# theblackcat102/edgedict

Hardware: NVIDIA H100
Metric: audio-sec/sec E6D2 B=32 T=1000 U=128 V=1024 training step (higher is better)
Workload: dtype bf16

## Files before the change

edgedict_b200/_lib.py:

```python
import ctypes as C
import os

_HERE = os.path.dirname(os.path.abspath(__file__))
LIB_PATH = os.path.join(_HERE, "libedgedict_b200.so")

_lib = None

P, I, L, F, D, Z = C.c_void_p, C.c_int, C.c_long, C.c_float, C.c_double, C.c_size_t

OPT_MAX_GROUPS = 16


class OptHyper(C.Structure):
    _fields_ = [(k, D * OPT_MAX_GROUPS) for k in ("lr", "wd", "b1", "b2", "eps")]


SIGNATURES = {
    "eb_rnnt_workspace_bytes": (Z, [I, I, I, I]),
    "eb_rnnt_loss_fwd": (I, [P, P, P, P, I, I, I, I, I, I, P, P, I, P]),
    "eb_rnnt_loss_bwd": (I, [P, P, I, P, P, P, I, I, I, I, I, I, P, P, I, D, P]),
    "eb_rnnt_loss_lattice": (I, [P, P, I, I, I, P, P, I, P]),
    "eb_rnnt_loss_bwd_bf16": (I, [P, P, P, P, P, I, I, I, I, I, P, P, I, D, P]),
    "eb_joint_logits_lse": (I, [P, P, P, P, P, P, P, P, P, P, I, I, I, I, I, I, P]),
    "eb_lm_logits_ce": (I, [P, P, P, P, P, I, P, P, L, I, I, P]),
    "eb_lm_ce_rows": (I, [P, P, I, P, P, L, I, P]),
    "eb_lm_ce_loss": (I, [P, P, P, I, L, L, I, I, P, P, P, P]),
    "eb_lm_ce_bwd": (I, [P, P, I, P, P, I, L, L, I, P, I, P, P]),
    "eb_rnnt_workspace_views": (I, [P, I, I, I, I, P, P, P, P, P]),
    "eb_rnnt_align_bytes": (Z, [I, I, I]),
    "eb_rnnt_viterbi": (I, [P, P, I, I, I, I, P, P, P, P, P, P]),
    "eb_log_softmax_fwd": (I, [P, P, L, I, P]),
    "eb_log_softmax_bwd": (I, [P, P, P, L, I, P]),
    "eb_ctc_workspace_size": (Z, [I, I, I]),
    "eb_ctc_loss_fwd": (I, [P, L, L, I, I, I, P, L, P, P, P, I, I, I, P, P, P]),
    "eb_ctc_loss_bwd": (I, [P, L, L, P, L, L, I, I, I, P, P, I, I, I, P, P, P]),
    "eb_ctc_greedy": (I, [P, L, L, I, I, I, P, I, P, P, P, P]),
    "eb_ctc_align_workspace_size": (Z, [I, I, I]),
    "eb_ctc_align": (I, [P, L, L, I, I, I, P, L, P, P, P, I, I, P, P, P, P]),
    "eb_gemm_f32": (I, [P, L, L, P, L, L, P, L, P, I, I, I, F, F, P]),
    "eb_gemm_bf16": (I, [P, I, P, I, P, I, P, I, L, I, L, P]),
    "eb_gemm_bf16_ex": (I, [P, I, P, I, P, I, P, I, L, I, L, I, P, L, P]),
    "eb_gemm_bf16_partials": (L, [I, I, I, L, I, L, I]),
    "eb_gemm_bf16_dtanh": (I, [P, I, P, I, P, P, L, I, L, P]),
    "eb_gemm_tc_set_trace": (I, [P, I]),
    "eb_joint_dpre_reduce": (I, [P, P, P, I, I, I, I, P]),
    "eb_lstm_scratch_bytes": (Z, [I, I]),
    "eb_lstm_seq_fwd": (I, [P, P, P, P, P, P, P, P, P, P, I, I, I, P]),
    "eb_lstm_seq_bwd": (I, [P, P, P, P, P, P, P, P, P, P, P, I, I, I, P]),
    "eb_gru_scratch_bytes": (Z, [I, I]),
    "eb_gru_seq_fwd": (I, [P, P, P, P, P, P, P, P, I, I, I, P]),
    "eb_gru_seq_bwd": (I, [P, P, P, P, P, P, P, P, P, P, I, I, I, P]),
    "eb_gru_tc_supported": (I, [I, I]),
    "eb_gru_tc_scratch_bytes": (Z, [I, I]),
    "eb_gru_tc_fwd": (I, [P, P, P, P, P, P, P, P, I, I, I, P]),
    "eb_gru_tc_bwd": (I, [P, P, P, P, P, P, P, P, P, P, I, I, I, P]),
# ... 103 lines not shown
```

edgedict_b200/csrc/common.cuh:

```cuda
#pragma once
#include <cuda_runtime.h>
#include <cuda_bf16.h>
#include <stdint.h>
#include <stdio.h>
#include <math.h>

#define EB_OK 0
#define EB_ERR_INVALID 2
#define EB_ERR_CUDA 3

#define EB_API extern "C" __attribute__((visibility("default")))

#define EB_CHECK_LAUNCH()                                                             \
    do {                                                                              \
        cudaError_t e__ = cudaGetLastError();                                         \
        if (e__ != cudaSuccess) {                                                     \
            fprintf(stderr, "[edgedict_b200] %s:%d CUDA error: %s\n", __FILE__,       \
                    __LINE__, cudaGetErrorString(e__));                               \
            return EB_ERR_CUDA;                                                       \
        }                                                                             \
    } while (0)

#define EB_CUDA(call)                                                                 \
    do {                                                                              \
// ... 50 lines not shown
    const int lane = threadIdx.x & 31, w = threadIdx.x >> 5;
    v = warp_sum(v);
    __syncthreads();
    if (lane == 0) sh[w] = v;
    __syncthreads();
    const int nw = (blockDim.x + 31) >> 5;
    T r = (threadIdx.x < nw) ? sh[threadIdx.x] : T(0);
    if (w == 0) {
        r = warp_sum(r);
        if (lane == 0) sh[32] = r;
    }
    __syncthreads();
    return sh[32];
}

__device__ __forceinline__ void spin_wait_ge(const unsigned* ctr, unsigned target) {
    unsigned v;
    long long t0 = 0;
    unsigned spins = 0;
    while (true) {
        asm volatile("ld.acquire.gpu.global.u32 %0, [%1];" : "=r"(v) : "l"(ctr) : "memory");
        if (v >= target) break;
        if ((++spins & 0xFFFF) == 0) {
            const long long now = clock64();
            if (t0 == 0) t0 = now;
            else if (now - t0 > 8000000000LL) {
                printf("[edgedict_b200] grid barrier timeout: block %d saw %u, wants %u\n", blockIdx.x, v, target);
                __trap();
            }
        }
    }
}

__device__ __forceinline__ float fast_ex2(float x) {
    float y;
    asm("ex2.approx.ftz.f32 %0, %1;" : "=f"(y) : "f"(x));
    return y;
}
__device__ __forceinline__ float fast_exp(float x) { return fast_ex2(x * 1.4426950408889634f); }
__device__ __forceinline__ float sigmoidf_(float x) { return 1.0f / (1.0f + expf(-x)); }

__device__ __forceinline__ float4 ld_stream_f4(const float* p) {
    float4 r;
    asm volatile("ld.global.nc.L1::no_allocate.v4.f32 {%0,%1,%2,%3}, [%4];"
                 : "=f"(r.x), "=f"(r.y), "=f"(r.z), "=f"(r.w) : "l"(p));
    return r;
}
__device__ __forceinline__ void st_stream_f4(float* p, float4 v) {
    asm volatile("st.global.L1::no_allocate.v4.f32 [%0], {%1,%2,%3,%4};"
                 :: "l"(p), "f"(v.x), "f"(v.y), "f"(v.z), "f"(v.w) : "memory");
}
```

edgedict_b200/csrc/elementwise.cu:

```cuda
#include <cooperative_groups.h>
#include "common.cuh"
#include "../../include/edgedict_b200.h"

namespace cg = cooperative_groups;

namespace {

constexpr int LN_WARPS = 8;

template <int PL>
__global__ void __launch_bounds__(LN_WARPS * 32)
layernorm_fwd_kernel(const float* __restrict__ x, const float* __restrict__ res,
                     const float* __restrict__ gamma, const float* __restrict__ beta,
                     float* __restrict__ y, __nv_bfloat16* __restrict__ y16,
                     float* __restrict__ mean, float* __restrict__ rstd, long rows, int H, float eps) {
    const int lane = threadIdx.x & 31;
    const long wstride = (long)gridDim.x * LN_WARPS;
    for (long r = (long)blockIdx.x * LN_WARPS + (threadIdx.x >> 5); r < rows; r += wstride) {
        const float* xr = x + r * H;
        const float* rr = res ? res + r * H : nullptr;
        float v[PL];
        float s = 0.f;
#pragma unroll
        for (int i = 0; i < PL; ++i) {
// ... 382 lines not shown
                acc[2 * i] += gf.x;
                acc[2 * i + 1] += gf.y;
            }
        }
        float* o = ddp + ((long)b * U + u) * J + q * 8;
        *reinterpret_cast<float4*>(o) = make_float4(acc[0], acc[1], acc[2], acc[3]);
        *reinterpret_cast<float4*>(o + 4) = make_float4(acc[4], acc[5], acc[6], acc[7]);
    }
}

template <int RL, int CW>
__device__ __forceinline__ float colsum_tree(float (*sh)[CW + 1], float v, int k, int cx) {
    sh[k][cx] = v;
    __syncthreads();
#pragma unroll 1
    for (int st = RL / 2; st > 0; st >>= 1) {
        if (k < st) sh[k][cx] += sh[k + st][cx];
        __syncthreads();
    }
    return sh[0][cx];
}
template <typename TI>
__global__ void __launch_bounds__(1024) colsum_kernel(const TI* __restrict__ x, float* __restrict__ out, long rows, int N) {
    __shared__ float sh[32][33];
    const int cx = threadIdx.x & 31, k = threadIdx.x >> 5;
    const int c = blockIdx.x * 32 + cx;
    float acc = 0.f;
    if (c < N)
        for (long r = k; r < rows; r += 32) acc += (float)x[r * N + c];
    const float t = colsum_tree<32, 32>(sh, acc, k, cx);
    if (k == 0 && c < N) out[c] += t;
}

constexpr int COLSUM_LANES = 512, COLSUM_CL = 4, COLSUM_CTA_LANES = COLSUM_LANES / COLSUM_CL;
__global__ void __cluster_dims__(1, COLSUM_CL, 1) __launch_bounds__(2 * COLSUM_CTA_LANES)
colsum_bf16_vec_kernel(const __nv_bfloat16* __restrict__ x, float* __restrict__ out, long rows, int N) {
    __shared__ float sh[COLSUM_CTA_LANES][17];
    cg::cluster_group cluster = cg::this_cluster();
    const unsigned rank = cluster.block_rank();
    const int half = threadIdx.x & 1, kl = threadIdx.x >> 1, k = (int)rank * COLSUM_CTA_LANES + kl;
    const int c0 = blockIdx.x * 16 + half * 8;
    float acc[8] = {0.f, 0.f, 0.f, 0.f, 0.f, 0.f, 0.f, 0.f};
    if (c0 < N) {
        const __nv_bfloat16* p = x + (long)k * N + c0;
        const long step = (long)COLSUM_LANES * N;
        long r = k;
        for (; r + 7 * COLSUM_LANES < rows; r += 8 * COLSUM_LANES) {
            uint4 v[8];
#pragma unroll
            for (int q = 0; q < 8; ++q) v[q] = *reinterpret_cast<const uint4*>(p + q * step);
#pragma unroll
            for (int q = 0; q < 8; ++q) {
                const uint32_t w[4] = {v[q].x, v[q].y, v[q].z, v[q].w};
#pragma unroll
                for (int i = 0; i < 4; ++i) {
                    const float2 f = __bfloat1622float2(*reinterpret_cast<const __nv_bfloat162*>(&w[i]));
                    acc[2 * i] += f.x;
                    acc[2 * i + 1] += f.y;
                }
            }
            p += 8 * step;
        }
        for (; r < rows; r += COLSUM_LANES, p += step) {
            const uint4 v = *reinterpret_cast<const uint4*>(p);
            const uint32_t w[4] = {v.x, v.y, v.z, v.w};
#pragma unroll
            for (int i = 0; i < 4; ++i) {
                const float2 f = __bfloat1622float2(*reinterpret_cast<const __nv_bfloat162*>(&w[i]));
                acc[2 * i] += f.x;
                acc[2 * i + 1] += f.y;
            }
        }
    }
#pragma unroll
    for (int i = 0; i < 8; ++i) sh[kl][half * 8 + i] = acc[i];
    cluster.sync();
    if (rank < 2) {
        const float* peer = cluster.map_shared_rank(&sh[0][0], rank + 2);
        for (int e = threadIdx.x; e < COLSUM_CTA_LANES * 16; e += blockDim.x) sh[e >> 4][e & 15] += peer[(e >> 4) * 17 + (e & 15)];
    }
    cluster.sync();
    if (rank == 0) {
        const float* peer = cluster.map_shared_rank(&sh[0][0], 1);
        for (int e = threadIdx.x; e < COLSUM_CTA_LANES * 16; e += blockDim.x) sh[e >> 4][e & 15] += peer[(e >> 4) * 17 + (e & 15)];
    }
    cluster.sync();
    if (rank != 0) return;
#pragma unroll 1
    for (int st = COLSUM_CTA_LANES / 2; st > 0; st >>= 1) {
        for (int e = threadIdx.x; e < st * 16; e += blockDim.x) sh[e >> 4][e & 15] += sh[(e >> 4) + st][e & 15];
        __syncthreads();
    }
    if (threadIdx.x < 16 && blockIdx.x * 16 + (int)threadIdx.x < N) out[blockIdx.x * 16 + threadIdx.x] += sh[0][threadIdx.x];
}

__global__ void cast_bf16_kernel(const float* __restrict__ x, __nv_bfloat16* __restrict__ y, long n) {
    long i = ((long)blockIdx.x * blockDim.x + threadIdx.x) * 4;
    const long stride = (long)gridDim.x * blockDim.x * 4;
    for (; i + 3 < n; i += stride) {
        float4 v = *reinterpret_cast<const float4*>(x + i);
        __nv_bfloat162 a = __floats2bfloat162_rn(v.x, v.y), b = __floats2bfloat162_rn(v.z, v.w);
        uint2 q;
        q.x = *reinterpret_cast<uint32_t*>(&a);
        q.y = *reinterpret_cast<uint32_t*>(&b);
        *reinterpret_cast<uint2*>(y + i) = q;
    }
    if (i < n) for (long k = i; k < n && k < i + 4; ++k) y[k] = __float2bfloat16(x[k]);
}

template <typename TI>
__global__ void transpose_to_bf16_kernel(const TI* __restrict__ x, __nv_bfloat16* __restrict__ y,
                                         long rows, long cols) {
    __shared__ float tile[32][33];
    const long c0 = (long)blockIdx.x * 32;
    for (long r0 = (long)blockIdx.y * 32; r0 < rows; r0 += (long)gridDim.y * 32) {
        for (int i = threadIdx.y; i < 32; i += blockDim.y) {
            long r = r0 + i, c = c0 + threadIdx.x;
            tile[i][threadIdx.x] = (r < rows && c < cols) ? (float)x[r * cols + c] : 0.f;
        }
        __syncthreads();
        for (int i = threadIdx.y; i < 32; i += blockDim.y) {
            long c = c0 + i, r = r0 + threadIdx.x;
            if (r < rows && c < cols) y[c * rows + r] = __float2bfloat16(tile[threadIdx.x][i]);
        }
        __syncthreads();
    }
// ... 199 lines not shown
    } else {
        joint_hidden_bwd_t_f32_kernel<<<B * T, 256, 0, ST(stream)>>>(
            (float*)dhidden_inout, (const float*)hidden, dep, T, U, J);
        EB_CHECK_LAUNCH();
        joint_hidden_bwd_u_f32_kernel<<<B * U, 256, 0, ST(stream)>>>((const float*)dhidden_inout, ddp, T, U, J);
    }
    EB_CHECK_LAUNCH();
    return EB_OK;
}

EB_API int eb_joint_dpre_reduce(const void* dpre16, float* dep, float* ddp, int B, int T, int U, int J, void* stream) {
    if (!dpre16 || !dep || !ddp || B <= 0 || T <= 0 || U <= 0 || J <= 0 || J % 8 ||
        ((reinterpret_cast<uintptr_t>(dpre16) | reinterpret_cast<uintptr_t>(dep) | reinterpret_cast<uintptr_t>(ddp)) & 15))
        return EB_ERR_INVALID;
    joint_dep_reduce_bf16_kernel<<<B * T, 96, 0, ST(stream)>>>((const __nv_bfloat16*)dpre16, dep, U, J);
    EB_CHECK_LAUNCH();
    joint_hidden_bwd_u_bf16_kernel<<<B * U, 96, 0, ST(stream)>>>((const __nv_bfloat16*)dpre16, ddp, T, U, J);
    EB_CHECK_LAUNCH();
    return EB_OK;
}

EB_API int eb_colsum(const void* x, int x_bf16, float* out, long rows, int N, void* stream) {
    if (!x || !out || rows <= 0 || N <= 0) return EB_ERR_INVALID;
    if (x_bf16 && N % 8 == 0 && (reinterpret_cast<uintptr_t>(x) & 15) == 0)
        colsum_bf16_vec_kernel<<<dim3((N + 15) / 16, COLSUM_CL), 2 * COLSUM_CTA_LANES, 0, ST(stream)>>>((const __nv_bfloat16*)x, out, rows, N);
    else if (x_bf16)
        colsum_kernel<__nv_bfloat16><<<(N + 31) / 32, 1024, 0, ST(stream)>>>((const __nv_bfloat16*)x, out, rows, N);
    else
        colsum_kernel<float><<<(N + 31) / 32, 1024, 0, ST(stream)>>>((const float*)x, out, rows, N);
    EB_CHECK_LAUNCH();
    return EB_OK;
}

EB_API int eb_cast_bf16(const float* x, void* y, long n, void* stream) {
    if (n <= 0) return EB_OK;
    if ((reinterpret_cast<uintptr_t>(x) & 15) || (reinterpret_cast<uintptr_t>(y) & 7)) return EB_ERR_INVALID;
    cast_bf16_kernel<<<ew_grid((n + 3) / 4, 256), 256, 0, ST(stream)>>>(x, (__nv_bfloat16*)y, n);
    EB_CHECK_LAUNCH();
    return EB_OK;
}

EB_API int eb_transpose_to_bf16(const void* x, int x_bf16, void* y, long rows, long cols, void* stream) {
    if (rows < 0 || cols < 0 || (cols + 31) / 32 > 0x7fffffffL) return EB_ERR_INVALID;
    if (rows == 0 || cols == 0) return EB_OK;
    if (!x || !y) return EB_ERR_INVALID;
    const long row_tiles = (rows + 31) / 32;
    dim3 grid((unsigned)((cols + 31) / 32), (unsigned)(row_tiles < 65535 ? row_tiles : 65535));
    if (x_bf16)
        transpose_to_bf16_kernel<__nv_bfloat16><<<grid, dim3(32, 8), 0, ST(stream)>>>(
            (const __nv_bfloat16*)x, (__nv_bfloat16*)y, rows, cols);
    else
        transpose_to_bf16_kernel<float><<<grid, dim3(32, 8), 0, ST(stream)>>>((const float*)x, (__nv_bfloat16*)y, rows, cols);
    EB_CHECK_LAUNCH();
    return EB_OK;
}

EB_API int eb_adam_step(float* p, const float* g, float* m, float* v, long n, float lr, float beta1,
                        float beta2, float eps, float weight_decay, int step, float grad_scale,
                        void* stream) {
    if (!p || !g || !m || !v || n <= 0 || step < 1) return EB_ERR_INVALID;
    float bc1 = 1.f - powf(beta1, (float)step), bc2 = 1.f - powf(beta2, (float)step);
    adam_kernel<<<ew_grid(n, 256), 256, 0, ST(stream)>>>(p, g, m, v, n, lr, beta1, beta2, eps,
                                                         weight_decay, bc1, bc2, grad_scale);
    EB_CHECK_LAUNCH();
    return EB_OK;
}
// ... 21 lines not shown
```

edgedict_b200/csrc/loss.cu:

```cuda
#include <atomic>

#include "common.cuh"
#include "../../include/rnnt.h"
#include "../../include/edgedict_b200.h"

namespace {

template <typename T> struct M;
template <> struct M<float> {
    static __device__ __forceinline__ float exp_fast(float x) { return fast_exp(x); }
    static __device__ __forceinline__ float exp_acc(float x) { return expf(x); }
    static __device__ __forceinline__ float log_acc(float x) { return logf(x); }
    static __device__ __forceinline__ float log1p_acc(float x) { return log1pf(x); }
    static __device__ __forceinline__ float ninf() { return -INFINITY; }
};
template <> struct M<double> {
    static __device__ __forceinline__ double exp_fast(double x) { return exp(x); }
    static __device__ __forceinline__ double exp_acc(double x) { return exp(x); }
    static __device__ __forceinline__ double log_acc(double x) { return log(x); }
    static __device__ __forceinline__ double log1p_acc(double x) { return log1p(x); }
    static __device__ __forceinline__ double ninf() { return -(double)INFINITY; }
};

template <typename T>
// ... 365 lines not shown
                    for (int i = 0; i < 4 && v + i < V; ++i) orow[v + i] = TO(T(0));
                }
            }
            continue;
        }
        const T sc = hscale * (gscale ? gscale[gscale_per_batch ? b : 0] : T(1));
        const T a = alphas[cell], bt_ = betas[cell], ll = ll_fwd[b], d = denom[cell];
        const int lab = (u < Un - 1) ? labels[b * (maxU - 1) + u] : -1;
        const T c_all = a + bt_ - ll + d;
        T c_blank = M<T>::ninf();
        if (t < Tn - 1) c_blank = a - ll + d + betas[cell + maxU];
        else if (u == Un - 1) c_blank = a - ll + d;
        const T c_lab = (lab >= 0) ? a - ll + d + betas[cell + 1] : M<T>::ninf();
        for (int v = lane * 4; v < V; v += 128) {
            T x[4];
            Row4<TI, VEC>::load(row, v, V, x);
            T g[4];
#pragma unroll
            for (int i = 0; i < 4; ++i) {
                T gr = M<T>::exp_fast(c_all + x[i]);
                if (v + i == blank) gr -= M<T>::exp_acc(c_blank + x[i]);
                if (v + i == lab) gr -= M<T>::exp_acc(c_lab + x[i]);
                g[i] = gr * sc;
            }
            if (VEC) {
                Store4<TO>::st(orow + v, g);
            } else {
                for (int i = 0; i < 4 && v + i < V; ++i) orow[v + i] = TO(g[i]);
            }
        }
    }
}

template <int WARPS>
__global__ void __launch_bounds__(WARPS * 32)
rnnt_grad_bf16x8_kernel(const __nv_bfloat16* logits, __nv_bfloat16* grads, const int* __restrict__ labels,
                        const int* __restrict__ xlen, const int* __restrict__ ylen, const float* __restrict__ denom,
                        const float* __restrict__ alphas, const float* __restrict__ betas,
                        const float* __restrict__ ll_fwd, const float* __restrict__ gscale, int gscale_per_batch,
                        float hscale, int B, int maxT, int maxU, int V, int blank) {
    const int lane = threadIdx.x & 31;
    const long ncells = (long)B * maxT * maxU;
    const long wstride = (long)gridDim.x * WARPS;
    for (long cell = (long)blockIdx.x * WARPS + (threadIdx.x >> 5); cell < ncells; cell += wstride) {
        const int u = (int)(cell % maxU);
        const long bt = cell / maxU;
        const int t = (int)(bt % maxT);
        const int b = (int)(bt / maxT);
        const int Tn = clamp_T(xlen[b], maxT), Un = clamp_U(ylen[b], maxU);
        const __nv_bfloat16* row = logits + cell * (long)V;
        __nv_bfloat16* orow = grads + cell * (long)V;
        if (t >= Tn || u >= Un) {
            for (int v = lane * 8; v < V; v += 256) *reinterpret_cast<uint4*>(orow + v) = make_uint4(0u, 0u, 0u, 0u);
            continue;
        }
        const float sc = hscale * (gscale ? gscale[gscale_per_batch ? b : 0] : 1.f);
        const float a = alphas[cell], bt_ = betas[cell], ll = ll_fwd[b], d = denom[cell];
        const int lab = (u < Un - 1) ? labels[b * (maxU - 1) + u] : -1;
        const float c_all = a + bt_ - ll + d;
        float c_blank = -INFINITY;
        if (t < Tn - 1) c_blank = a - ll + d + betas[cell + maxU];
        else if (u == Un - 1) c_blank = a - ll + d;
        const float c_lab = (lab >= 0) ? a - ll + d + betas[cell + 1] : -INFINITY;
        constexpr float LOG2E = 1.4426950408889634f;
        const float c2 = c_all * LOG2E;
        for (int v0 = lane * 8; v0 < V; v0 += 1024) {
            uint4 qq[4];
#pragma unroll
            for (int k = 0; k < 4; ++k)
                if (v0 + k * 256 < V) qq[k] = *reinterpret_cast<const uint4*>(row + v0 + k * 256);
#pragma unroll
            for (int k = 0; k < 4; ++k) {
                const int v = v0 + k * 256;
                if (v >= V) break;
                const uint32_t w[4] = {qq[k].x, qq[k].y, qq[k].z, qq[k].w};
                float x[8], g[8];
#pragma unroll
                for (int i = 0; i < 4; ++i) {
                    const float2 f = __bfloat1622float2(*reinterpret_cast<const __nv_bfloat162*>(&w[i]));
                    x[2 * i] = f.x; x[2 * i + 1] = f.y;
                }
#pragma unroll
                for (int i = 0; i < 8; ++i) g[i] = fast_ex2(fmaf(x[i], LOG2E, c2));
                const unsigned ib = (unsigned)(blank - v), il = (unsigned)(lab - v);
                if (ib < 8u || il < 8u) {
#pragma unroll
                    for (int i = 0; i < 8; ++i) {
                        if ((unsigned)i == ib) g[i] -= expf(c_blank + x[i]);
                        if ((unsigned)i == il) g[i] -= expf(c_lab + x[i]);
                    }
                }
                uint32_t ow[4];
#pragma unroll
                for (int i = 0; i < 4; ++i) {
                    __nv_bfloat162 pk = __floats2bfloat162_rn(g[2 * i] * sc, g[2 * i + 1] * sc);
                    ow[i] = *reinterpret_cast<uint32_t*>(&pk);
                }
                *reinterpret_cast<uint4*>(orow + v) = make_uint4(ow[0], ow[1], ow[2], ow[3]);
            }
        }
    }
}

template <typename T>
struct Workspace {
    T *denom, *lpb, *lpl, *alphas, *betas, *ll_fwd, *ll_bwd;
    static size_t bytes(int B, int maxT, int maxU) {
        return sizeof(T) * ((size_t)B * maxT * maxU * 5 + 2 * (size_t)B);
    }
    Workspace(void* ws, int B, int maxT, int maxU) {
        const size_t n = (size_t)B * maxT * maxU;
        T* p = reinterpret_cast<T*>(ws);
        denom = p; lpb = p + n; lpl = p + 2 * n; alphas = p + 3 * n; betas = p + 4 * n;
        ll_fwd = p + 5 * n; ll_bwd = ll_fwd + B;
    }
};

template <typename T>
int launch_lattice(const Workspace<T>& w, const int* xlen, const int* ylen, int B, int maxT, int maxU, int need_beta,
                   cudaStream_t st) {
    static std::atomic<int> cache[64];
    int dev;
    EB_CUDA(cudaGetDevice(&dev));
    int narrow_max = dev < 64 ? cache[dev].load(std::memory_order_relaxed) : 0;
    if (!narrow_max) {
        cudaFuncAttributes a;
        EB_CUDA(cudaFuncGetAttributes(&a, rnnt_lattice_kernel<T>));
        narrow_max = a.maxThreadsPerBlock;
        if (dev < 64) cache[dev].store(narrow_max, std::memory_order_relaxed);
    }
    const int threads = ((maxU + 31) / 32) * 32;
    const size_t smem = 2 * threads * sizeof(T);
    if (threads <= narrow_max)
        rnnt_lattice_kernel<T><<<dim3(B, 2), threads, smem, st>>>(w.lpb, w.lpl, xlen, ylen, w.alphas, w.betas,
// ... 255 lines not shown
}

EB_API int eb_rnnt_loss_bwd_bf16(const void* logits16, void* grads16, const int* labels, const int* xlen,
                                 const int* ylen, int B, int maxT, int maxU, int V, int blank, void* workspace,
                                 const float* gscale_dev, int gscale_per_batch, double host_scale, void* stream) {
    if (!logits16 || !grads16 || !workspace || bad_problem(labels, xlen, ylen, B, maxT, maxU, V, blank))
        return EB_ERR_INVALID;
    cudaStream_t st = reinterpret_cast<cudaStream_t>(stream);
    Workspace<float> w(workspace, B, maxT, maxU);
    const long ncells = (long)B * maxT * maxU;
    constexpr int WARPS = 8;
    const bool vec = (V % 4 == 0) && ((reinterpret_cast<uintptr_t>(logits16) & 7) == 0) &&
                     ((reinterpret_cast<uintptr_t>(grads16) & 7) == 0);
    const __nv_bfloat16* in = reinterpret_cast<const __nv_bfloat16*>(logits16);
    __nv_bfloat16* out = reinterpret_cast<__nv_bfloat16*>(grads16);
    const bool vec8 = (V % 8 == 0) && ((reinterpret_cast<uintptr_t>(logits16) & 15) == 0) &&
                      ((reinterpret_cast<uintptr_t>(grads16) & 15) == 0);
    if (vec8)
        rnnt_grad_bf16x8_kernel<WARPS><<<row_grid(ncells, WARPS), WARPS * 32, 0, st>>>(
            in, out, labels, xlen, ylen, w.denom, w.alphas, w.betas, w.ll_fwd, gscale_dev, gscale_per_batch,
            (float)host_scale, B, maxT, maxU, V, blank);
    else if (vec)
        rnnt_grad_kernel<float, __nv_bfloat16, true, WARPS, __nv_bfloat16><<<row_grid(ncells, WARPS), WARPS * 32, 0, st>>>(
            in, out, labels, xlen, ylen, w.denom, w.alphas, w.betas, w.ll_fwd, gscale_dev, gscale_per_batch,
            (float)host_scale, B, maxT, maxU, V, blank);
    else
        rnnt_grad_kernel<float, __nv_bfloat16, false, WARPS, __nv_bfloat16><<<row_grid(ncells, WARPS), WARPS * 32, 0, st>>>(
            in, out, labels, xlen, ylen, w.denom, w.alphas, w.betas, w.ll_fwd, gscale_dev, gscale_per_batch,
            (float)host_scale, B, maxT, maxU, V, blank);
    EB_CHECK_LAUNCH();
    return EB_OK;
}

EB_API int eb_rnnt_workspace_views(void* workspace, int B, int maxT, int maxU, int dtype_size,
                                   void** denom, void** alphas, void** betas, void** ll_fwd,
                                   void** ll_bwd) {
    if (dtype_size == 4) {
        Workspace<float> w(workspace, B, maxT, maxU);
        *denom = w.denom; *alphas = w.alphas; *betas = w.betas; *ll_fwd = w.ll_fwd; *ll_bwd = w.ll_bwd;
    } else {
        Workspace<double> w(workspace, B, maxT, maxU);
        *denom = w.denom; *alphas = w.alphas; *betas = w.betas; *ll_fwd = w.ll_fwd; *ll_bwd = w.ll_bwd;
    }
    return EB_OK;
}
```

edgedict_b200/functional.py:

```python
import torch

from . import ops

import os

f32, bf16 = torch.float32, torch.bfloat16
FUSE_JOINT_LSE = os.environ.get("EDGEDICT_FUSE_LSE", "1") != "0"


def _c(t):
    return t if t.is_contiguous() else t.contiguous()


class Linear(torch.autograd.Function):

    @staticmethod
    def forward(ctx, x, w, b, precision):
        shp = x.shape
        x2 = _c(x).view(-1, shp[-1])
        x16 = ops.cast_bf16(x2) if precision == "bf16" else None
        y = ops.mm_nt(x2, w, b, precision, x16=x16)
        ctx.save_for_backward(x2 if x16 is None else x16, w)
        ctx.precision, ctx.has_b, ctx.shp = precision, b is not None, shp
        return y.view(*shp[:-1], w.shape[0])
# ... 773 lines not shown
    def forward(ctx, h_enc, h_dec, w1, b1, w2, b2, labels, act_lens, label_lens, blank, precision):
        B, T, E = h_enc.shape
        U, Dd = h_dec.shape[1], h_dec.shape[2]
        J, V = w1.shape[0], w2.shape[0]
        he2, hd2, ep, dp = _joint_pre(h_enc, h_dec, w1, b1, precision)
        hid = ops.joint_hidden_fwd(ep, dp, precision == "bf16")
        hid2 = hid.view(B * T * U, J)
        fused = _fused_lse(precision, J, U)
        if fused:
            b2a = b2 if (b2.is_contiguous() and b2.data_ptr() % 16 == 0) else b2.clone()
            logits, ws = ops.joint_logits_lse(hid2, ops.cast_bf16(w2.contiguous()), b2a, labels, act_lens,
                                              label_lens, B, T, U, blank)
            costs = ops.rnnt_lattice(act_lens, label_lens, B, T, U, ws)
        else:
            logits = ops.mm_nt(hid2, w2, b2, precision, x16=hid2 if precision == "bf16" else None).view(B, T, U, V)
            costs, ws = ops.rnnt_loss_fwd(logits, labels, act_lens, label_lens, blank, need_beta=True)
        ctx.save_for_backward(hid, he2, hd2, w1, w2, logits, labels, act_lens, label_lens, ws)
        ctx.precision, ctx.dims, ctx.blank = precision, (B, T, U, E, Dd, J, V), blank
        ctx.mark_non_differentiable(costs)
        loss = costs.sum().unsqueeze(-1) / B
        ctx.costs = costs
        return loss, costs

    @staticmethod
    def backward(ctx, go, _gc):
        hid, he2, hd2, w1, w2, logits, labels, act_lens, label_lens, ws = ctx.saved_tensors
        if getattr(ctx, "consumed", False):
            raise RuntimeError("JointLoss.backward ran twice on the same graph: the gradient is written in place over "
                               "the saved logits (retain_graph is not supported by this node)")
        ctx.consumed = True
        B, T, U, E, Dd, J, V = ctx.dims
        p = ctx.precision
        g = _c(go.to(f32)).view(-1)
        if logits.dtype == bf16:
            dl = ops.rnnt_loss_bwd_bf16(logits, labels, act_lens, label_lens, ctx.blank, ws, g, 1.0 / B)
        elif p == "bf16":
            dl = ops.rnnt_loss_bwd(logits, labels, act_lens, label_lens, ctx.blank, ws, g, 1.0 / B, out_bf16=True)
        else:
            dl = ops.rnnt_loss_bwd(logits, labels, act_lens, label_lens, ctx.blank, ws, g, 1.0 / B, out=logits)
        dhe, dhd, dw1, db1, dw2, db2 = _joint_bwd(p, dl.view(B * T * U, V), hid, he2, hd2, w1, w2, ctx.dims)
        return dhe, dhd, dw1, db1, dw2, db2, None, None, None, None, None


def conv_out_len(T, k, s):
    return (T + k - 2) // s + 2 - k


class FrontEndStack(torch.autograd.Function):

    @staticmethod
    def forward(ctx, x, spec, precision, *params):
        first, blocks, ln_eps = spec
        bf = precision == "bf16"
        B = x.shape[0]
        it = iter(params)
        saves, meta = [], []
        if first is not None:
            k, s, C, hb = first
            w0 = next(it)
            b0 = next(it) if hb else None
            T = conv_out_len(x.shape[1], k, s)
            y = ops.conv1d_first_fwd(x, _c(w0.view(C, k)), b0, k, s, T)
        else:
            y, T, C = x, x.shape[1], x.shape[2]
        ustride = T * C
        for (k, s, Cin, Cout, hb, eps) in blocks:
            w = next(it)
            b = next(it) if hb else None
            g, be = next(it), next(it)
            mean, rstd = ops.gn_stats(y, ustride, B, T, Cin, eps)
            Q = (k - 1 + T + s - 1) // s
            rows = B * Q + (k + s - 1) // s
            xp = torch.empty(rows * s * Cin, dtype=bf16 if bf else f32, device=x.device)
# ... 229 lines not shown
```

edgedict_b200/ops.py:

```python
import torch

from ._lib import lib
from ._lib import check as _check


def _s():
    return torch.cuda.current_stream().cuda_stream


def _p(t):
    if t is None:
        return None
    if not t.is_cuda:
        raise RuntimeError("edgedict_b200 ops need CUDA tensors (got a %s tensor); there is no CPU path" % t.device)
    return t.data_ptr()


def _need(t, dtype=None, name="tensor"):
    if not t.is_cuda:
        raise RuntimeError("edgedict_b200 ops need CUDA tensors (%s is on %s); there is no CPU path" % (name, t.device))
    if dtype is not None and t.dtype != dtype:
        raise TypeError("%s must be %s, got %s" % (name, dtype, t.dtype))
    if not t.is_contiguous():
        raise ValueError("%s must be contiguous" % name)
    return t


f32, bf16 = torch.float32, torch.bfloat16


class _Prof:

    def __init__(self):
        self.enabled = False
        self.events = []
        self.launches = 0

    def reset(self):
        self.events, self.launches = [], 0

    def summary(self, base=None):
        out, spans = {}, {}
        for name, a, b, nbytes, flops in self.events:
            d = out.setdefault(name, dict(ms=0.0, ms_sum=0.0, calls=0, bytes=0.0, flops=0.0))
            d["ms_sum"] += a.elapsed_time(b)
            d["calls"] += 1
            d["bytes"] += nbytes
            d["flops"] += flops
            if base is not None:
                spans.setdefault(name, []).append((base.elapsed_time(a), base.elapsed_time(b)))
        for name, d in out.items():
            if base is None:
                d["ms"] = d["ms_sum"]
                continue
            tot, cur_s, cur_e = 0.0, None, None
            for s0, e0 in sorted(spans[name]):
                if cur_e is None or s0 > cur_e:
                    if cur_e is not None:
                        tot += cur_e - cur_s
                    cur_s, cur_e = s0, e0
                else:
# ... 536 lines not shown
    return logits16, ws


def rnnt_lattice(xlen, ylen, B, T, U, ws, need_beta=True):
    costs = torch.empty(B, dtype=f32, device=ws.device)
    with _timed("rnnt_loss_fwd", 2, 0.0, 0.0):
        check(lib().eb_rnnt_loss_lattice(_p(xlen), _p(ylen), B, T, U, _p(ws), _p(costs), int(need_beta), _s()),
              "eb_rnnt_loss_lattice")
    return costs


def rnnt_viterbi(xlen, ylen, B, T, U, ws, dtype):
    dev = ws.device
    dec = torch.empty(lib().eb_rnnt_align_bytes(B, T, U), dtype=torch.uint8, device=dev)
    frames = torch.empty(B, U - 1, dtype=torch.int32, device=dev)
    label_logp = torch.empty(B, U - 1, dtype=dtype, device=dev)
    score = torch.empty(B, dtype=dtype, device=dev)
    with _timed("rnnt_viterbi", 1, 0.0, 0.0):
        check(lib().eb_rnnt_viterbi(_p(xlen), _p(ylen), B, T, U, 8 if dtype == torch.float64 else 4, _p(ws),
                                    _p(dec) if dec.numel() else None, _p(frames), _p(label_logp), _p(score), _s()),
              "eb_rnnt_viterbi")
    return frames, label_logp, score


def rnnt_loss_bwd_bf16(logits16, labels, xlen, ylen, blank, ws, gscale, host_scale):
    B, T, U, V = logits16.shape
    per_batch = int(gscale is not None and gscale.numel() > 1)
    with _timed("rnnt_loss_bwd", 1, 4.0 * B * T * U * V, 0.0):
        check(lib().eb_rnnt_loss_bwd_bf16(_p(logits16), _p(logits16), _p(labels), _p(xlen), _p(ylen), B, T, U, V, blank,
                                          _p(ws), _p(gscale), per_batch, float(host_scale), _s()), "eb_rnnt_loss_bwd_bf16")
    return logits16


def _targets(t):
    _need(t, None, "targets")
    if t.dtype not in (torch.int32, torch.int64):
        raise TypeError("targets must be int32 or int64, got %s" % t.dtype)
    return int(t.dtype == torch.int64)


def lm_logits_ce(hid16, w16, b, targets):
    M, K = hid16.shape
    V = w16.shape[0]
    t64 = _targets(targets)
    logits16 = torch.empty(M, V, dtype=bf16, device=hid16.device)
    lse = torch.empty(M, dtype=f32, device=hid16.device)
    tl = torch.empty(M, dtype=f32, device=hid16.device)
    with _timed("lm_logits_ce", 1, 2.0 * (M * K + V * K) + 2.0 * M * V, 2.0 * M * V * K):
        check(lib().eb_lm_logits_ce(_p(hid16), _p(w16), _p(b), _p(logits16), _p(targets), t64, _p(lse), _p(tl), M, V, K,
                                    _s()), "eb_lm_logits_ce")
    return logits16, lse, tl


def lm_ce_rows(logits, targets):
    _need(logits, f32, "logits")
    M, V = logits.shape
    t64 = _targets(targets)
    lse = torch.empty(M, dtype=f32, device=logits.device)
    tl = torch.empty(M, dtype=f32, device=logits.device)
    with _timed("lm_ce_rows", 1, 4.0 * M * V, 0.0):
        check(lib().eb_lm_ce_rows(_p(logits), _p(targets), t64, _p(lse), _p(tl), M, V, _s()), "eb_lm_ce_rows")
    return lse, tl


def lm_ce_loss(lse, tl, targets, ignore_index, V, mean):
    M = lse.shape[0]
# ... 376 lines not shown
```

include/edgedict_b200.h:

```cpp
#pragma once
#include <stddef.h>
#include <stdint.h>
#ifdef __cplusplus
extern "C" {
#endif

size_t eb_rnnt_workspace_bytes(int B, int maxT, int maxU, int dtype_size);
int eb_rnnt_loss_fwd(const void* logits, const int* labels, const int* xlen, const int* ylen,
                     int B, int maxT, int maxU, int V, int blank, int dtype_size,
                     void* workspace, void* costs_dev , int need_beta,
                     void* stream);
int eb_rnnt_loss_bwd(const void* logits, void* grads, int grads_bf16, const int* labels,
                     const int* xlen, const int* ylen, int B, int maxT, int maxU, int V, int blank,
                     int dtype_size, void* workspace, const void* gscale_dev ,
                     int gscale_per_batch, double host_scale, void* stream);
int eb_rnnt_loss_lattice(const int* xlen, const int* ylen, int B, int maxT, int maxU, void* workspace,
                         float* costs_dev, int need_beta, void* stream);
int eb_rnnt_loss_bwd_bf16(const void* logits16, void* grads16, const int* labels, const int* xlen, const int* ylen,
                          int B, int maxT, int maxU, int V, int blank, void* workspace, const float* gscale_dev,
                          int gscale_per_batch, double host_scale, void* stream);
int eb_rnnt_workspace_views(void* workspace, int B, int maxT, int maxU, int dtype_size,
                            void** denom, void** alphas, void** betas, void** ll_fwd, void** ll_bwd);
size_t eb_rnnt_align_bytes(int B, int maxT, int maxU);
int eb_rnnt_viterbi(const int* xlen, const int* ylen, int B, int maxT, int maxU, int dtype_size, const void* workspace,
                    void* decisions, int* frames, void* label_logp, void* score, void* stream);

int eb_log_softmax_fwd(const float* x, float* y, long rows, int V, void* stream);
int eb_log_softmax_bwd(const float* dy, const float* y, float* dx, long rows, int V, void* stream);
size_t eb_ctc_workspace_size(int N, int T, int S);
int eb_ctc_loss_fwd(const float* log_probs, long stride_n, long stride_t, int N, int T, int V, const int* targets,
                    long ntargets, const int* target_offsets, const int* target_lengths, const int* input_lengths,
                    int S, int blank, int zero_infinity, void* workspace, float* costs, void* stream);
int eb_ctc_loss_bwd(const float* log_probs, long stride_n, long stride_t, float* grad, long grad_stride_n,
                    long grad_stride_t, int N, int T, int V, const int* target_lengths, const int* input_lengths,
                    int S, int blank, int zero_infinity, const void* workspace, const float* gscale, void* stream);
int eb_ctc_greedy(const float* log_probs, long stride_b, long stride_t, int B, int T, int V, const int* xlen, int blank,
                  int* ids, int* counts, float* neg_score, void* stream);
size_t eb_ctc_align_workspace_size(int B, int T, int S);
int eb_ctc_align(const float* log_probs, long stride_b, long stride_t, int B, int T, int V, const int* targets,
                 long ntargets, const int* tg_off, const int* tg_len, const int* in_len, int S, int blank, void* workspace,
                 int* alignment, float* frame_logp, void* stream);

int eb_gemm_f32(const float* A, long sam, long sak, const float* B, long sbk, long sbn, float* C,
                long ldc, const float* bias, int M, int N, int K, float alpha, float beta,
                void* stream);

int eb_gemm_bf16(const void* A, int a_mn_major, const void* B, int b_mn_major, void* C, int c_bf16,
                 const float* bias, int accumulate, long M, int N, long K, void* stream);

#define EB_GEMM_CORESIDENT 1
#define EB_GEMM_FIXED_K 2
long eb_gemm_bf16_partials(int a_mn_major, int c_bf16, int accumulate, long M, int N, long K, int flags);
int eb_gemm_bf16_ex(const void* A, int a_mn_major, const void* B, int b_mn_major, void* C, int c_bf16,
// ... 197 lines not shown
```

Measured before the change: 13880.

## Fuse joint output-bias gradient column sum into RNN-T bf16 loss backward

Adds a new RNN-T bf16 gradient kernel that also accumulates per-lane partial column sums of the produced gradient, followed by a small finish kernel that reduces the partials into the output-bias gradient. This removes the separate pass that re-reads the full B*T*U*V gradient tensor to compute db2. The kernel switches from a warp-per-row layout to a thread-per-8-columns layout that strides over rows, which changes memory coalescing and parallelism. It relies on _joint_bwd accepting a precomputed db2 and skipping its own column sum.

```diff
diff --git a/edgedict_b200/_lib.py b/edgedict_b200/_lib.py
--- a/edgedict_b200/_lib.py
+++ b/edgedict_b200/_lib.py
@@ -21,6 +21,7 @@
     "eb_rnnt_loss_bwd": (I, [P, P, I, P, P, P, I, I, I, I, I, I, P, P, I, D, P]),
     "eb_rnnt_loss_lattice": (I, [P, P, I, I, I, P, P, I, P]),
     "eb_rnnt_loss_bwd_bf16": (I, [P, P, P, P, P, I, I, I, I, I, P, P, I, D, P]),
+    "eb_rnnt_loss_bwd_bf16_db": (I, [P, P, P, P, P, I, I, I, I, I, P, P, I, D, P, P, P]),
     "eb_joint_logits_lse": (I, [P, P, P, P, P, P, P, P, P, P, I, I, I, I, I, I, P]),
     "eb_lm_logits_ce": (I, [P, P, P, P, P, I, P, P, L, I, I, P]),
     "eb_lm_ce_rows": (I, [P, P, I, P, P, L, I, P]),
diff --git a/edgedict_b200/csrc/common.cuh b/edgedict_b200/csrc/common.cuh
--- a/edgedict_b200/csrc/common.cuh
+++ b/edgedict_b200/csrc/common.cuh
@@ -106,6 +106,9 @@
     }
 }
 
+constexpr int COLSUM_LANES = 512;
+int colsum_lanes_finish(const float* part, float* out, int N, cudaStream_t st);
+
 __device__ __forceinline__ float fast_ex2(float x) {
     float y;
     asm("ex2.approx.ftz.f32 %0, %1;" : "=f"(y) : "f"(x));
diff --git a/edgedict_b200/csrc/elementwise.cu b/edgedict_b200/csrc/elementwise.cu
--- a/edgedict_b200/csrc/elementwise.cu
+++ b/edgedict_b200/csrc/elementwise.cu
@@ -438,7 +438,7 @@
     if (k == 0 && c < N) out[c] += t;
 }
 
-constexpr int COLSUM_LANES = 512, COLSUM_CL = 4, COLSUM_CTA_LANES = COLSUM_LANES / COLSUM_CL;
+constexpr int COLSUM_CL = 4, COLSUM_CTA_LANES = COLSUM_LANES / COLSUM_CL;
 __global__ void __cluster_dims__(1, COLSUM_CL, 1) __launch_bounds__(2 * COLSUM_CTA_LANES)
 colsum_bf16_vec_kernel(const __nv_bfloat16* __restrict__ x, float* __restrict__ out, long rows, int N) {
     __shared__ float sh[COLSUM_CTA_LANES][17];
@@ -498,6 +498,21 @@
         __syncthreads();
     }
     if (threadIdx.x < 16 && blockIdx.x * 16 + (int)threadIdx.x < N) out[blockIdx.x * 16 + threadIdx.x] += sh[0][threadIdx.x];
+}
+
+__global__ void __launch_bounds__(COLSUM_LANES) colsum_lanes_finish_kernel(const float* __restrict__ part,
+                                                                           float* __restrict__ out, int N) {
+    __shared__ float sh[COLSUM_LANES][17];
+    const int c0 = blockIdx.x * 16;
+    for (int e = threadIdx.x; e < COLSUM_LANES * 16; e += blockDim.x)
+        sh[e >> 4][e & 15] = c0 + (e & 15) < N ? part[(long)(e >> 4) * N + c0 + (e & 15)] : 0.f;
+    __syncthreads();
+#pragma unroll 1
+    for (int st = COLSUM_LANES / 2; st > 0; st >>= 1) {
+        for (int e = threadIdx.x; e < st * 16; e += blockDim.x) sh[e >> 4][e & 15] += sh[(e >> 4) + st][e & 15];
+        __syncthreads();
+    }
+    if (threadIdx.x < 16 && c0 + (int)threadIdx.x < N) out[c0 + threadIdx.x] += sh[0][threadIdx.x];
 }
 
 __global__ void cast_bf16_kernel(const float* __restrict__ x, __nv_bfloat16* __restrict__ y, long n) {
@@ -763,6 +778,12 @@
     return EB_OK;
 }
 
+int colsum_lanes_finish(const float* part, float* out, int N, cudaStream_t st) {
+    colsum_lanes_finish_kernel<<<(N + 15) / 16, COLSUM_LANES, 0, st>>>(part, out, N);
+    EB_CHECK_LAUNCH();
+    return EB_OK;
+}
+
 EB_API int eb_cast_bf16(const float* x, void* y, long n, void* stream) {
     if (n <= 0) return EB_OK;
     if ((reinterpret_cast<uintptr_t>(x) & 15) || (reinterpret_cast<uintptr_t>(y) & 7)) return EB_ERR_INVALID;
diff --git a/edgedict_b200/csrc/loss.cu b/edgedict_b200/csrc/loss.cu
--- a/edgedict_b200/csrc/loss.cu
+++ b/edgedict_b200/csrc/loss.cu
@@ -421,6 +421,81 @@
     }
 }
 
+struct GradRow {
+    float c2, c_blank, c_lab, sc;
+    int lab;
+    bool pad;
+};
+
+__device__ __forceinline__ void cell_btu(long cell, int maxT, int maxU, int& b, int& t, int& u) {
+    u = (int)(cell % maxU);
+    const long bt = cell / maxU;
+    t = (int)(bt % maxT);
+    b = (int)(bt / maxT);
+}
+
+struct GradLoads {
+    float a, bt_, ll, d, gs, b_next, b_lab;
+    int lab;
+};
+
+__device__ __forceinline__ GradLoads grad_loads(long cell, int b, int t, int u, int Tn, int Un,
+                                                const int* __restrict__ labels, const float* __restrict__ denom,
+                                                const float* __restrict__ alphas, const float* __restrict__ betas,
+                                                const float* __restrict__ ll_fwd, const float* __restrict__ gscale,
+                                                int gscale_per_batch, int maxU) {
+    GradLoads l;
+    l.gs = gscale ? gscale[gscale_per_batch ? b : 0] : 1.f;
+    l.a = alphas[cell]; l.bt_ = betas[cell]; l.ll = ll_fwd[b]; l.d = denom[cell];
+    l.lab = (u < Un - 1) ? labels[b * (maxU - 1) + u] : -1;
+    l.b_next = (t < Tn - 1) ? betas[cell + maxU] : 0.f;
+    l.b_lab = (u < Un - 1) ? betas[cell + 1] : 0.f;
+    return l;
+}
+
+__device__ __forceinline__ GradRow grad_row(const GradLoads& l, int t, int u, int Tn, int Un, float hscale) {
+    GradRow r;
+    r.pad = t >= Tn || u >= Un;
+    r.sc = hscale * l.gs;
+    r.lab = l.lab;
+    const float c_all = l.a + l.bt_ - l.ll + l.d;
+    r.c_blank = -INFINITY;
+    if (t < Tn - 1) r.c_blank = l.a - l.ll + l.d + l.b_next;
+    else if (u == Un - 1) r.c_blank = l.a - l.ll + l.d;
+    r.c_lab = (r.lab >= 0) ? l.a - l.ll + l.d + l.b_lab : -INFINITY;
+    constexpr float LOG2E = 1.4426950408889634f;
+    r.c2 = c_all * LOG2E;
+    return r;
+}
+
+__device__ __forceinline__ uint4 grad_bf16x8(uint4 q, int v, const GradRow& r, int blank) {
+    constexpr float LOG2E = 1.4426950408889634f;
+    const uint32_t w[4] = {q.x, q.y, q.z, q.w};
+    float x[8], g[8];
+#pragma unroll
+    for (int i = 0; i < 4; ++i) {
+        const float2 f = __bfloat1622float2(*reinterpret_cast<const __nv_bfloat162*>(&w[i]));
+        x[2 * i] = f.x; x[2 * i + 1] = f.y;
+    }
+#pragma unroll
+    for (int i = 0; i < 8; ++i) g[i] = fast_ex2(fmaf(x[i], LOG2E, r.c2));
+    const unsigned ib = (unsigned)(blank - v), il = (unsigned)(r.lab - v);
+    if (ib < 8u || il < 8u) {
+#pragma unroll
+        for (int i = 0; i < 8; ++i) {
+            if ((unsigned)i == ib) g[i] -= expf(r.c_blank + x[i]);
+            if ((unsigned)i == il) g[i] -= expf(r.c_lab + x[i]);
+        }
+    }
+    uint32_t ow[4];
+#pragma unroll
+    for (int i = 0; i < 4; ++i) {
+        __nv_bfloat162 pk = __floats2bfloat162_rn(g[2 * i] * r.sc, g[2 * i + 1] * r.sc);
+        ow[i] = *reinterpret_cast<uint32_t*>(&pk);
+    }
+    return make_uint4(ow[0], ow[1], ow[2], ow[3]);
+}
+
 template <int WARPS>
 __global__ void __launch_bounds__(WARPS * 32)
 rnnt_grad_bf16x8_kernel(const __nv_bfloat16* logits, __nv_bfloat16* grads, const int* __restrict__ labels,
@@ -432,27 +507,19 @@
     const long ncells = (long)B * maxT * maxU;
     const long wstride = (long)gridDim.x * WARPS;
     for (long cell = (long)blockIdx.x * WARPS + (threadIdx.x >> 5); cell < ncells; cell += wstride) {
-        const int u = (int)(cell % maxU);
-        const long bt = cell / maxU;
-        const int t = (int)(bt % maxT);
-        const int b = (int)(bt / maxT);
+        int b, t, u;
+        cell_btu(cell, maxT, maxU, b, t, u);
         const int Tn = clamp_T(xlen[b], maxT), Un = clamp_U(ylen[b], maxU);
+        const bool pad = t >= Tn || u >= Un;
+        const GradRow r = grad_row(pad ? GradLoads{} : grad_loads(cell, b, t, u, Tn, Un, labels, denom, alphas, betas,
+                                                                  ll_fwd, gscale, gscale_per_batch, maxU),
+                                   t, u, Tn, Un, hscale);
         const __nv_bfloat16* row = logits + cell * (long)V;
         __nv_bfloat16* orow = grads + cell * (long)V;
-        if (t >= Tn || u >= Un) {
+        if (r.pad) {
             for (int v = lane * 8; v < V; v += 256) *reinterpret_cast<uint4*>(orow + v) = make_uint4(0u, 0u, 0u, 0u);
             continue;
         }
-        const float sc = hscale * (gscale ? gscale[gscale_per_batch ? b : 0] : 1.f);
-        const float a = alphas[cell], bt_ = betas[cell], ll = ll_fwd[b], d = denom[cell];
-        const int lab = (u < Un - 1) ? labels[b * (maxU - 1) + u] : -1;
-        const float c_all = a + bt_ - ll + d;
-        float c_blank = -INFINITY;
-        if (t < Tn - 1) c_blank = a - ll + d + betas[cell + maxU];
-        else if (u == Un - 1) c_blank = a - ll + d;
-        const float c_lab = (lab >= 0) ? a - ll + d + betas[cell + 1] : -INFINITY;
-        constexpr float LOG2E = 1.4426950408889634f;
-        const float c2 = c_all * LOG2E;
         for (int v0 = lane * 8; v0 < V; v0 += 1024) {
             uint4 qq[4];
 #pragma unroll
@@ -462,33 +529,63 @@
             for (int k = 0; k < 4; ++k) {
                 const int v = v0 + k * 256;
                 if (v >= V) break;
-                const uint32_t w[4] = {qq[k].x, qq[k].y, qq[k].z, qq[k].w};
-                float x[8], g[8];
-#pragma unroll
-                for (int i = 0; i < 4; ++i) {
-                    const float2 f = __bfloat1622float2(*reinterpret_cast<const __nv_bfloat162*>(&w[i]));
-                    x[2 * i] = f.x; x[2 * i + 1] = f.y;
-                }
-#pragma unroll
-                for (int i = 0; i < 8; ++i) g[i] = fast_ex2(fmaf(x[i], LOG2E, c2));
-                const unsigned ib = (unsigned)(blank - v), il = (unsigned)(lab - v);
-                if (ib < 8u || il < 8u) {
-#pragma unroll
-                    for (int i = 0; i < 8; ++i) {
-                        if ((unsigned)i == ib) g[i] -= expf(c_blank + x[i]);
-                        if ((unsigned)i == il) g[i] -= expf(c_lab + x[i]);
-                    }
-                }
-                uint32_t ow[4];
-#pragma unroll
-                for (int i = 0; i < 4; ++i) {
-                    __nv_bfloat162 pk = __floats2bfloat162_rn(g[2 * i] * sc, g[2 * i + 1] * sc);
-                    ow[i] = *reinterpret_cast<uint32_t*>(&pk);
-                }
-                *reinterpret_cast<uint4*>(orow + v) = make_uint4(ow[0], ow[1], ow[2], ow[3]);
-            }
-        }
-    }
+                *reinterpret_cast<uint4*>(orow + v) = grad_bf16x8(qq[k], v, r, blank);
+            }
+        }
+    }
+}
+
+constexpr int DB_THREADS = 128, DB_ROWS = 4;
+__global__ void __launch_bounds__(DB_THREADS, 4)
+rnnt_grad_db_bf16x8_kernel(const __nv_bfloat16* logits, __nv_bfloat16* grads, const int* __restrict__ labels,
+                           const int* __restrict__ xlen, const int* __restrict__ ylen, const float* __restrict__ denom,
+                           const float* __restrict__ alphas, const float* __restrict__ betas,
+                           const float* __restrict__ ll_fwd, const float* __restrict__ gscale, int gscale_per_batch,
+                           float hscale, int B, int maxT, int maxU, int V, int blank, float* __restrict__ part) {
+    const int V8 = V / 8;
+    const int tid = blockIdx.x * DB_THREADS + threadIdx.x;
+    if (tid >= COLSUM_LANES * V8) return;
+    const int k = tid / V8, v = (tid - k * V8) * 8;
+    const long ncells = (long)B * maxT * maxU;
+    float acc[8] = {0.f, 0.f, 0.f, 0.f, 0.f, 0.f, 0.f, 0.f};
+    for (long c0 = k; c0 < ncells; c0 += (long)DB_ROWS * COLSUM_LANES) {
+        int bi[DB_ROWS], ti[DB_ROWS], ui[DB_ROWS], Tn[DB_ROWS], Un[DB_ROWS];
+#pragma unroll
+        for (int i = 0; i < DB_ROWS; ++i) {
+            const long cell = c0 + (long)i * COLSUM_LANES;
+            cell_btu(cell < ncells ? cell : ncells - 1, maxT, maxU, bi[i], ti[i], ui[i]);
+            Tn[i] = clamp_T(xlen[bi[i]], maxT);
+            Un[i] = cell < ncells ? clamp_U(ylen[bi[i]], maxU) : 0;
+        }
+        GradLoads l[DB_ROWS];
+        uint4 q[DB_ROWS];
+#pragma unroll
+        for (int i = 0; i < DB_ROWS; ++i) {
+            const long cell = c0 + (long)i * COLSUM_LANES;
+            const long cl = cell < ncells ? cell : ncells - 1;
+            l[i] = grad_loads(cl, bi[i], ti[i], ui[i], Tn[i], Un[i], labels, denom, alphas, betas, ll_fwd, gscale,
+                              gscale_per_batch, maxU);
+            if (ti[i] < Tn[i] && ui[i] < Un[i]) q[i] = *reinterpret_cast<const uint4*>(logits + cell * (long)V + v);
+        }
+#pragma unroll
+        for (int i = 0; i < DB_ROWS; ++i) {
+            const long cell = c0 + (long)i * COLSUM_LANES;
+            if (cell >= ncells) break;
+            const GradRow r = grad_row(l[i], ti[i], ui[i], Tn[i], Un[i], hscale);
+            const uint4 g = r.pad ? make_uint4(0u, 0u, 0u, 0u) : grad_bf16x8(q[i], v, r, blank);
+            *reinterpret_cast<uint4*>(grads + cell * (long)V + v) = g;
+            const uint32_t w[4] = {g.x, g.y, g.z, g.w};
+#pragma unroll
+            for (int j = 0; j < 4; ++j) {
+                const float2 f = __bfloat1622float2(*reinterpret_cast<const __nv_bfloat162*>(&w[j]));
+                acc[2 * j] += f.x;
+                acc[2 * j + 1] += f.y;
+            }
+        }
+    }
+    float* o = part + (long)k * V + v;
+    *reinterpret_cast<float4*>(o) = make_float4(acc[0], acc[1], acc[2], acc[3]);
+    *reinterpret_cast<float4*>(o + 4) = make_float4(acc[4], acc[5], acc[6], acc[7]);
 }
 
 template <typename T>
@@ -810,6 +907,26 @@
     return EB_OK;
 }
 
+EB_API int eb_rnnt_loss_bwd_bf16_db(const void* logits16, void* grads16, const int* labels, const int* xlen,
+                                    const int* ylen, int B, int maxT, int maxU, int V, int blank, void* workspace,
+                                    const float* gscale_dev, int gscale_per_batch, double host_scale, float* db_part,
+                                    float* db_accum, void* stream) {
+    if (!logits16 || !grads16 || !workspace || !db_part || !db_accum ||
+        bad_problem(labels, xlen, ylen, B, maxT, maxU, V, blank) || V % 8 ||
+        ((reinterpret_cast<uintptr_t>(logits16) | reinterpret_cast<uintptr_t>(grads16) |
+          reinterpret_cast<uintptr_t>(db_part)) & 15))
+        return EB_ERR_INVALID;
+    cudaStream_t st = reinterpret_cast<cudaStream_t>(stream);
+    Workspace<float> w(workspace, B, maxT, maxU);
+    const int threads = COLSUM_LANES * (V / 8);
+    rnnt_grad_db_bf16x8_kernel<<<(threads + DB_THREADS - 1) / DB_THREADS, DB_THREADS, 0, st>>>(
+        reinterpret_cast<const __nv_bfloat16*>(logits16), reinterpret_cast<__nv_bfloat16*>(grads16), labels, xlen, ylen,
+        w.denom, w.alphas, w.betas, w.ll_fwd, gscale_dev, gscale_per_batch, (float)host_scale, B, maxT, maxU, V, blank,
+        db_part);
+    EB_CHECK_LAUNCH();
+    return colsum_lanes_finish(db_part, db_accum, V, st);
+}
+
 EB_API int eb_rnnt_workspace_views(void* workspace, int B, int maxT, int maxU, int dtype_size,
                                    void** denom, void** alphas, void** betas, void** ll_fwd,
                                    void** ll_bwd) {
diff --git a/edgedict_b200/functional.py b/edgedict_b200/functional.py
--- a/edgedict_b200/functional.py
+++ b/edgedict_b200/functional.py
@@ -829,13 +829,16 @@
         B, T, U, E, Dd, J, V = ctx.dims
         p = ctx.precision
         g = _c(go.to(f32)).view(-1)
-        if logits.dtype == bf16:
+        db2 = None
+        if logits.dtype == bf16 and V % 8 == 0:
+            dl, db2 = ops.rnnt_loss_bwd_bf16_db(logits, labels, act_lens, label_lens, ctx.blank, ws, g, 1.0 / B)
+        elif logits.dtype == bf16:
             dl = ops.rnnt_loss_bwd_bf16(logits, labels, act_lens, label_lens, ctx.blank, ws, g, 1.0 / B)
         elif p == "bf16":
             dl = ops.rnnt_loss_bwd(logits, labels, act_lens, label_lens, ctx.blank, ws, g, 1.0 / B, out_bf16=True)
         else:
             dl = ops.rnnt_loss_bwd(logits, labels, act_lens, label_lens, ctx.blank, ws, g, 1.0 / B, out=logits)
-        dhe, dhd, dw1, db1, dw2, db2 = _joint_bwd(p, dl.view(B * T * U, V), hid, he2, hd2, w1, w2, ctx.dims)
+        dhe, dhd, dw1, db1, dw2, db2 = _joint_bwd(p, dl.view(B * T * U, V), hid, he2, hd2, w1, w2, ctx.dims, db2)
         return dhe, dhd, dw1, db1, dw2, db2, None, None, None, None, None
 
 
diff --git a/edgedict_b200/ops.py b/edgedict_b200/ops.py
--- a/edgedict_b200/ops.py
+++ b/edgedict_b200/ops.py
@@ -27,6 +27,7 @@
 
 
 f32, bf16 = torch.float32, torch.bfloat16
+COLSUM_LANES = 512
 
 
 class _Prof:
@@ -629,6 +630,18 @@
     return logits16
 
 
+def rnnt_loss_bwd_bf16_db(logits16, labels, xlen, ylen, blank, ws, gscale, host_scale):
+    B, T, U, V = logits16.shape
+    per_batch = int(gscale is not None and gscale.numel() > 1)
+    part = torch.empty(COLSUM_LANES * V, dtype=f32, device=logits16.device)
+    db = torch.zeros(V, dtype=f32, device=logits16.device)
+    with _timed("rnnt_loss_bwd", 2, 4.0 * B * T * U * V, 0.0):
+        check(lib().eb_rnnt_loss_bwd_bf16_db(_p(logits16), _p(logits16), _p(labels), _p(xlen), _p(ylen), B, T, U, V,
+                                             blank, _p(ws), _p(gscale), per_batch, float(host_scale), _p(part), _p(db),
+                                             _s()), "eb_rnnt_loss_bwd_bf16_db")
+    return logits16, db
+
+
 def _targets(t):
     _need(t, None, "targets")
     if t.dtype not in (torch.int32, torch.int64):
diff --git a/include/edgedict_b200.h b/include/edgedict_b200.h
--- a/include/edgedict_b200.h
+++ b/include/edgedict_b200.h
@@ -19,6 +19,9 @@
 int eb_rnnt_loss_bwd_bf16(const void* logits16, void* grads16, const int* labels, const int* xlen, const int* ylen,
                           int B, int maxT, int maxU, int V, int blank, void* workspace, const float* gscale_dev,
                           int gscale_per_batch, double host_scale, void* stream);
+int eb_rnnt_loss_bwd_bf16_db(const void* logits16, void* grads16, const int* labels, const int* xlen, const int* ylen,
+                             int B, int maxT, int maxU, int V, int blank, void* workspace, const float* gscale_dev,
+                             int gscale_per_batch, double host_scale, float* db_part, float* db_accum, void* stream);
 int eb_rnnt_workspace_views(void* workspace, int B, int maxT, int maxU, int dtype_size,
                             void** denom, void** alphas, void** betas, void** ll_fwd, void** ll_bwd);
 size_t eb_rnnt_align_bytes(int B, int maxT, int maxU);
```

After: 14460 (median of 6 runs). +4.2%, better.
